# marja-w/gan-des-midi-music-gen

Measured on AMD Instinct MI355X. Metric: GAN training samples/sec (G+D step), higher is better.
Workload: dtype bf16; 1 GPU; SIMNN G/D iteration, synthetic 128x256 spectrogram windows; per_gpu_batch=256, global_batch=256, mode=faithful, parallelism=dp1

## Files before the change

### gan_des_midi_music_gen_amd/csrc/pointwise.hip

```cpp
#include "gdm_common.h"
#include "adam_pc.h"

namespace {

__global__ __launch_bounds__(1024) void bce_kernel(const float* __restrict__ x, float target, int n, float gscale,
                                                   float* __restrict__ loss, float* __restrict__ dx, int fuse_sig,
                                                   int accumulate) {
  __shared__ float red[1024];
  const int t = threadIdx.x;
  float s = 0.f;
  for (int i = t; i < n; i += 1024) {
    const float v = x[i];
    s += fmaxf(v, 0.f) - v * target + log1pf(expf(-fabsf(v)));
    if (dx) {
      float g = (1.0f / (1.0f + expf(-v)) - target) * gscale / (float)n;
      if (fuse_sig) g *= v * (1.f - v);
      dx[i] = g;
    }
  }
  red[t] = s;
  __syncthreads();
  for (int o = 512; o > 0; o >>= 1) {
    if (t < o) red[t] += red[t + o];
    __syncthreads();
// ... 67 lines not shown
                   blockIdx.z);
}

template <bool VEC>
__global__ __launch_bounds__(256) void adam_dev_kernel(float* __restrict__ p, const float* __restrict__ g,
                                                       float* __restrict__ m, float* __restrict__ v, int64_t n,
                                                       const float* __restrict__ hyper) {
  const float w1 = 1.0f - hyper[2], beta2 = hyper[3], omb2 = 1.0f - hyper[3], eps = hyper[4], gscale = hyper[5];
  const float step_size = hyper[6], bc2_sqrt = hyper[7];
  const int64_t stride = (int64_t)gridDim.x * 256 * 4;
  for (int64_t i = ((int64_t)blockIdx.x * 256 + threadIdx.x) * 4; i < n; i += stride) {
    if (VEC && i + 3 < n) {
      f32x4 pp = *(const f32x4*)(p + i), gg = *(const f32x4*)(g + i), mm = *(const f32x4*)(m + i),
            vv = *(const f32x4*)(v + i);
#pragma unroll
      for (int j = 0; j < 4; ++j) {
        float pj = pp[j], mj = mm[j], vj = vv[j];
        adam_element(pj, mj, vj, gg[j], gscale, w1, beta2, omb2, eps, step_size, bc2_sqrt);
        pp[j] = pj; mm[j] = mj; vv[j] = vj;
      }
      *(f32x4*)(p + i) = pp;
      *(f32x4*)(m + i) = mm;
      *(f32x4*)(v + i) = vv;
    } else {
      for (int64_t k = i; k < n && k < i + 4; ++k) {
        adam_element(p[k], m[k], v[k], g[k], gscale, w1, beta2, omb2, eps, step_size, bc2_sqrt);
      }
    }
  }
}

struct Welford { float n, mean, m2; };
__device__ __forceinline__ void welford_merge(Welford& a, const Welford& b) {
  if (b.n == 0.f) return;
  const float n = a.n + b.n;
  const float d = b.mean - a.mean;
  a.mean += d * (b.n / n);
  a.m2 += b.m2 + d * d * (a.n * b.n / n);
  a.n = n;
}

__device__ __forceinline__ Welford welford_from_shifted(float n, float shift, float s, float ss) {
  Welford a{n, 0.f, 0.f};
  if (n > 0.f) {
    a.mean = shift + s / n;
    a.m2 = fmaxf(ss - s * (s / n), 0.f);
  }
  return a;
}

__global__ __launch_bounds__(256) void bn_partial_stats(const float* __restrict__ y, int rows, int C, int chunk_rows,
                                                        int CW, float* __restrict__ ws) {
  __shared__ Welford sh[4][64];
  const int lane = threadIdx.x & 63, wv = threadIdx.x >> 6;
  const int rpl = 64 / CW;
  const int c = blockIdx.x * 64 + (lane & (CW - 1)), sub = lane / CW;
  const int r0 = blockIdx.y * chunk_rows, r1 = min(rows, r0 + chunk_rows);
  const int step = 4 * rpl;
  float n = 0.f, shift = 0.f, s = 0.f, ss = 0.f;
  if (c < C) {
    int r = r0 + wv * rpl + sub;
    if (r < r1) shift = y[(int64_t)r * C + c];
    for (; r + 7 * step < r1; r += 8 * step) {
      float x[8];
#pragma unroll
      for (int q = 0; q < 8; ++q) x[q] = y[(int64_t)(r + q * step) * C + c];
#pragma unroll
      for (int q = 0; q < 8; ++q) { const float d = x[q] - shift; s += d; ss += d * d; }
      n += 8.f;
    }
    for (; r < r1; r += step) { const float d = y[(int64_t)r * C + c] - shift; s += d; ss += d * d; n += 1.f; }
  }
  sh[wv][lane] = welford_from_shifted(n, shift, s, ss);
  __syncthreads();
  if (wv == 0 && sub == 0 && c < C) {
    Welford t{0.f, 0.f, 0.f};
    for (int w = 0; w < 4; ++w)
      for (int q = 0; q < rpl; ++q) welford_merge(t, sh[w][q * CW + lane]);
    float* o = ws + ((int64_t)blockIdx.y * C + c) * 3;
    o[0] = t.n; o[1] = t.mean; o[2] = t.m2;
  }
}

__global__ __launch_bounds__(1024) void bn_finalize(const float* __restrict__ ws, int chunks, int rows, int C,
                                                    float momentum, float eps, float* __restrict__ running_mean,
                                                    float* __restrict__ running_var, int64_t* __restrict__ nbt,
                                                    float* __restrict__ save_mean, float* __restrict__ save_invstd) {
  __shared__ Welford part[16][64];
  const int lane = threadIdx.x & 63, wv = threadIdx.x >> 6;
  const int c = blockIdx.x * 64 + lane;
  if (blockIdx.x == 0 && threadIdx.x == 0 && nbt) nbt[0] += 1;
  Welford t{0.f, 0.f, 0.f};
  if (c < C)
    for (int k = wv; k < chunks; k += 16 * 8) {
      Welford b[8];
#pragma unroll
      for (int q = 0; q < 8; ++q) {
        const int kk = k + 16 * q;
        const float* o = ws + ((int64_t)min(kk, chunks - 1) * C + c) * 3;
        b[q] = Welford{kk < chunks ? o[0] : 0.f, o[1], o[2]};
      }
#pragma unroll
      for (int q = 0; q < 8; ++q) welford_merge(t, b[q]);
    }
  part[wv][lane] = t;
  __syncthreads();
  if (wv != 0 || c >= C) return;
  t = part[0][lane];
#pragma unroll
  for (int w = 1; w < 16; ++w) welford_merge(t, part[w][lane]);
  const float var_b = t.m2 / (float)rows;
  save_mean[c] = t.mean;
  save_invstd[c] = 1.0f / sqrtf(var_b + eps);
  if (running_mean) {
    const float var_u = t.m2 / (float)max(rows - 1, 1);
    running_mean[c] = (1.f - momentum) * running_mean[c] + momentum * t.mean;
    running_var[c] = (1.f - momentum) * running_var[c] + momentum * var_u;
  }
}

__global__ __launch_bounds__(256) void bn_eval_stats(const float* __restrict__ running_mean,
                                                     const float* __restrict__ running_var, int C, float eps,
                                                     float* __restrict__ save_mean, float* __restrict__ save_invstd) {
  const int c = blockIdx.x * 256 + threadIdx.x;
  if (c >= C) return;
  save_mean[c] = running_mean[c];
  save_invstd[c] = 1.0f / sqrtf(running_var[c] + eps);
}

template <typename IT>
__global__ __launch_bounds__(256) void bn_apply(const float* __restrict__ y, int64_t total64, int C,
                                                const float* __restrict__ gamma, const float* __restrict__ beta,
                                                const float* __restrict__ mean, const float* __restrict__ invstd,
                                                int act, void* __restrict__ out, int out_dtype) {
  const IT total = (IT)total64, stride = (IT)gridDim.x * 256;
  for (IT i = (IT)blockIdx.x * 256 + threadIdx.x; i < total; i += stride) {
    const int c = (int)(i % C);
    const float alpha = invstd[c] * gamma[c];
    const float v = (y[i] - mean[c]) * alpha + beta[c];
    store_from_f32(out, out_dtype, i, apply_act(v, act, 0.f));
  }
}

__global__ __launch_bounds__(256) void bn_bwd_partial(const void* __restrict__ dout, const void* __restrict__ out,
                                                      int dtype, const float* __restrict__ y, int rows, int C,
                                                      int chunk_rows, const float* __restrict__ mean,
                                                      const float* __restrict__ invstd, int act,
                                                      float* __restrict__ ws) {
  __shared__ float sh1[4][64], sh2[4][64];
  const int lane = threadIdx.x & 63, wv = threadIdx.x >> 6;
  const int c = blockIdx.x * 64 + lane;
  const int r0 = blockIdx.y * chunk_rows, r1 = min(rows, r0 + chunk_rows);
  float s1 = 0.f, s2 = 0.f;
  if (c < C) {
    const float mu = mean[c], is = invstd[c];
    for (int r = r0 + wv; r < r1; r += 4) {
      const int64_t i = (int64_t)r * C + c;
      const float g = load_as_f32(dout, dtype, i) * act_grad_from_out(load_as_f32(out, dtype, i), act, 0.f);
      s1 += g;
      s2 += g * ((y[i] - mu) * is);
    }
  }
  sh1[wv][lane] = s1; sh2[wv][lane] = s2;
  __syncthreads();
  if (wv == 0 && c < C) {
    float* o = ws + ((int64_t)blockIdx.y * C + c) * 2;
    o[0] = ((sh1[0][lane] + sh1[1][lane]) + sh1[2][lane]) + sh1[3][lane];
    o[1] = ((sh2[0][lane] + sh2[1][lane]) + sh2[2][lane]) + sh2[3][lane];
  }
}

__global__ __launch_bounds__(256) void bn_bwd_finalize(const float* __restrict__ ws, int chunks, int C,
                                                       float* __restrict__ dgamma, float* __restrict__ dbeta) {
  const int c = blockIdx.x * 256 + threadIdx.x;
  if (c >= C) return;
  float s1 = 0.f, s2 = 0.f;
  for (int k = 0; k < chunks; ++k) {
    s1 += ws[((int64_t)k * C + c) * 2];
    s2 += ws[((int64_t)k * C + c) * 2 + 1];
  }
  dbeta[c] = s1;
  dgamma[c] = s2;
}

__global__ __launch_bounds__(256) void bn_bwd_apply(const void* __restrict__ dout, const void* __restrict__ out,
                                                    int dtype, const float* __restrict__ y, int64_t total, int rows,
                                                    int C, const float* __restrict__ gamma,
                                                    const float* __restrict__ mean, const float* __restrict__ invstd,
                                                    const float* __restrict__ dgamma, const float* __restrict__ dbeta,
                                                    int act, float* __restrict__ dy) {
  const int64_t stride = (int64_t)gridDim.x * 256;
  const float inv_r = 1.0f / (float)rows;
  for (int64_t i = (int64_t)blockIdx.x * 256 + threadIdx.x; i < total; i += stride) {
    const int c = (int)(i % C);
    const float g = load_as_f32(dout, dtype, i) * act_grad_from_out(load_as_f32(out, dtype, i), act, 0.f);
    const float xhat = (y[i] - mean[c]) * invstd[c];
    dy[i] = gamma[c] * invstd[c] * (g - dbeta[c] * inv_r - xhat * dgamma[c] * inv_r);
  }
}

__global__ __launch_bounds__(256) void bias_act_kernel(const float* __restrict__ x, const float* __restrict__ bias,
// ... 86 lines not shown
  GDM_LAUNCH_OK("gdm_criterion_loss");
  return GDM_OK;
}

extern "C" int gdm_adam_step(float* p, const float* g, float* m, float* v, int64_t n, int step, float lr, float beta1,
                             float beta2, float eps, float grad_scale, void* stream) {
  GDM_REQUIRE(p && g && m && v, "gdm_adam_step: null pointer");
  GDM_REQUIRE(n > 0 && step >= 1, "gdm_adam_step: bad n=%lld or step=%d", (long long)n, step);
  const bool aligned = (((uintptr_t)p | (uintptr_t)g | (uintptr_t)m | (uintptr_t)v) & 15) == 0;
  const double bc1 = 1.0 - pow((double)beta1, (double)step);
  const double bc2 = 1.0 - pow((double)beta2, (double)step);
  const float step_size = (float)((double)lr / bc1);
  const float bc2_sqrt = (float)sqrt(bc2);
  int64_t blocks = (n / 4 + 255) / 256;
  if (blocks < 1) blocks = 1;
  if (blocks > 8192) blocks = 8192;
  if (aligned)
    hipLaunchKernelGGL(adam_kernel<true>, dim3((unsigned)blocks), dim3(256), 0, (hipStream_t)stream, p, g, m, v, n,
                       1.0f - beta1, beta2, 1.0f - beta2, step_size, bc2_sqrt, eps, grad_scale);
  else
    hipLaunchKernelGGL(adam_kernel<false>, dim3((unsigned)blocks), dim3(256), 0, (hipStream_t)stream, p, g, m, v, n,
                       1.0f - beta1, beta2, 1.0f - beta2, step_size, bc2_sqrt, eps, grad_scale);
  GDM_LAUNCH_OK("gdm_adam_step");
  return GDM_OK;
}

extern "C" int gdm_adam_step_dev_pc(float* p, const float* g_pc, float* m, float* v, int N, int C, int P,
                                    void* shadow_pc, int shadow_dtype, float* hyper, int advance_step, void* stream) {
  GDM_REQUIRE(p && g_pc && m && v && shadow_pc && hyper, "gdm_adam_step_dev_pc: null pointer");
  GDM_REQUIRE(N > 0 && C > 0 && P > 0 && N <= 65535 && (C + 31) / 32 <= 65535 && gdm_dtype_ok(shadow_dtype),
              "gdm_adam_step_dev_pc: bad arguments");
  hipStream_t s = (hipStream_t)stream;
  if (advance_step) hipLaunchKernelGGL(adam_prep_kernel, dim3(1), dim3(1), 0, s, hyper);
  const dim3 grid((P + 127) / 128, (C + 31) / 32, N);
  const int vec_ok = (P % 4 == 0) && ((((uintptr_t)p | (uintptr_t)m | (uintptr_t)v) & 15) == 0);
  if (shadow_dtype == GDM_BF16)
    hipLaunchKernelGGL(adam_dev_pc_kernel<__bf16>, grid, dim3(256), 0, s, p, g_pc, m, v, C, P, (__bf16*)shadow_pc, hyper,
                       vec_ok);
  else
    hipLaunchKernelGGL(adam_dev_pc_kernel<float>, grid, dim3(256), 0, s, p, g_pc, m, v, C, P, (float*)shadow_pc, hyper,
                       vec_ok);
  GDM_LAUNCH_OK("gdm_adam_step_dev_pc");
  return GDM_OK;
}

extern "C" int gdm_adam_step_dev(float* p, const float* g, float* m, float* v, int64_t n, float* hyper, void* stream) {
  GDM_REQUIRE(p && g && m && v && hyper && n > 0, "gdm_adam_step_dev: bad arguments");
  const bool aligned = (((uintptr_t)p | (uintptr_t)g | (uintptr_t)m | (uintptr_t)v) & 15) == 0;
  int64_t blocks = (n / 4 + 255) / 256;
  if (blocks < 1) blocks = 1;
  if (blocks > 8192) blocks = 8192;
  hipStream_t s = (hipStream_t)stream;
  hipLaunchKernelGGL(adam_prep_kernel, dim3(1), dim3(1), 0, s, hyper);
  if (aligned) hipLaunchKernelGGL(adam_dev_kernel<true>, dim3((unsigned)blocks), dim3(256), 0, s, p, g, m, v, n, hyper);
  else hipLaunchKernelGGL(adam_dev_kernel<false>, dim3((unsigned)blocks), dim3(256), 0, s, p, g, m, v, n, hyper);
  GDM_LAUNCH_OK("gdm_adam_step_dev");
  return GDM_OK;
}

extern "C" size_t gdm_bn_workspace_bytes(int rows, int channels) {
  return (size_t)row_chunks(rows) * (size_t)channels * 3 * sizeof(float);
}

extern "C" int gdm_bn_act_fwd(const float* y, int rows, int channels, const float* gamma, const float* beta,
                              float* running_mean, float* running_var, int64_t* num_batches_tracked, float momentum,
                              float eps, int act, void* out, int out_dtype, float* save_mean, float* save_invstd,
                              int training, void* workspace, size_t workspace_bytes, void* stream) {
  GDM_REQUIRE(y && gamma && beta && out && save_mean && save_invstd, "gdm_bn_act_fwd: null pointer");
  GDM_REQUIRE(rows > 0 && channels > 0 && gdm_dtype_ok(out_dtype), "gdm_bn_act_fwd: bad arguments");
  hipStream_t s = (hipStream_t)stream;
  const int C = channels;
  if (training) {
    GDM_REQUIRE(rows > 1, "gdm_bn_act_fwd: training-mode batch norm needs more than 1 value per channel");
    const int chunks = row_chunks(rows);
    if (!workspace || workspace_bytes < gdm_bn_workspace_bytes(rows, C)) {
      gdm_set_error("gdm_bn_act_fwd: workspace too small");
      return GDM_EWORKSPACE;
    }
    const int chunk_rows = (rows + chunks - 1) / chunks;
    int cw = 64;
    while (cw / 2 >= C && cw > 1) cw /= 2;
    hipLaunchKernelGGL(bn_partial_stats, dim3((C + 63) / 64, chunks), dim3(256), 0, s, y, rows, C, chunk_rows, cw,
                       (float*)workspace);
    hipLaunchKernelGGL(bn_finalize, dim3((C + 63) / 64), dim3(1024), 0, s, (const float*)workspace, chunks, rows, C,
                       momentum, eps, running_mean, running_var, num_batches_tracked, save_mean, save_invstd);
  } else {
    GDM_REQUIRE(running_mean && running_var, "gdm_bn_act_fwd: eval mode needs running statistics");
    hipLaunchKernelGGL(bn_eval_stats, dim3((C + 255) / 256), dim3(256), 0, s, running_mean, running_var, C, eps,
                       save_mean, save_invstd);
  }
  const int64_t total = (int64_t)rows * C;
  if (total < ((int64_t)1 << 31))
    hipLaunchKernelGGL(bn_apply<int>, dim3(grid_for(total)), dim3(256), 0, s, y, total, C, gamma, beta, save_mean,
                       save_invstd, act, out, out_dtype);
  else
    hipLaunchKernelGGL(bn_apply<int64_t>, dim3(grid_for(total)), dim3(256), 0, s, y, total, C, gamma, beta, save_mean,
                       save_invstd, act, out, out_dtype);
  GDM_LAUNCH_OK("gdm_bn_act_fwd");
  return GDM_OK;
}

extern "C" int gdm_bn_partial_chunks(int rows) { return row_chunks(rows); }

extern "C" int gdm_bn_partials(const float* y, int rows, int channels, float* partials, void* stream) {
  GDM_REQUIRE(y && partials && rows > 0 && channels > 0, "gdm_bn_partials: bad arguments");
  const int C = channels, chunks = row_chunks(rows), chunk_rows = (rows + chunks - 1) / chunks;
  int cw = 64;
  while (cw / 2 >= C && cw > 1) cw /= 2;
  hipLaunchKernelGGL(bn_partial_stats, dim3((C + 63) / 64, chunks), dim3(256), 0, (hipStream_t)stream, y, rows, C,
                     chunk_rows, cw, partials);
  GDM_LAUNCH_OK("gdm_bn_partials");
  return GDM_OK;
}

extern "C" int gdm_bn_apply(const float* y, int rows, int channels, const float* gamma, const float* beta,
                            const float* mean, const float* invstd, int act, void* out, int out_dtype, void* stream) {
  GDM_REQUIRE(y && gamma && beta && mean && invstd && out && rows > 0 && channels > 0 && gdm_dtype_ok(out_dtype),
              "gdm_bn_apply: bad arguments");
  const int64_t total = (int64_t)rows * channels;
  hipStream_t s = (hipStream_t)stream;
  if (total < ((int64_t)1 << 31))
    hipLaunchKernelGGL(bn_apply<int>, dim3(grid_for(total)), dim3(256), 0, s, y, total, channels, gamma, beta, mean, invstd,
                       act, out, out_dtype);
  else
    hipLaunchKernelGGL(bn_apply<int64_t>, dim3(grid_for(total)), dim3(256), 0, s, y, total, channels, gamma, beta, mean,
                       invstd, act, out, out_dtype);
  GDM_LAUNCH_OK("gdm_bn_apply");
  return GDM_OK;
}

extern "C" int gdm_bn_finalize(const float* ws, int chunks, int rows, int channels, float momentum, float eps,
                               float* running_mean, float* running_var, int64_t* num_batches_tracked, float* save_mean,
                               float* save_invstd, void* stream) {
  GDM_REQUIRE(ws && save_mean && save_invstd && chunks > 0 && rows > 1 && channels > 0, "gdm_bn_finalize: bad arguments");
  hipLaunchKernelGGL(bn_finalize, dim3((channels + 63) / 64), dim3(1024), 0, (hipStream_t)stream, ws, chunks, rows,
                     channels, momentum, eps, running_mean, running_var, num_batches_tracked, save_mean, save_invstd);
  GDM_LAUNCH_OK("gdm_bn_finalize");
  return GDM_OK;
}

extern "C" int gdm_bn_stats(const float* y, int rows, int channels, float* running_mean, float* running_var,
                            int64_t* num_batches_tracked, float momentum, float eps, float* save_mean,
                            float* save_invstd, void* workspace, size_t workspace_bytes, void* stream) {
  GDM_REQUIRE(y && save_mean && save_invstd && rows > 1 && channels > 0, "gdm_bn_stats: bad arguments");
  if (!workspace || workspace_bytes < gdm_bn_workspace_bytes(rows, channels)) {
    gdm_set_error("gdm_bn_stats: workspace too small");
    return GDM_EWORKSPACE;
  }
  hipStream_t s = (hipStream_t)stream;
  const int C = channels, chunks = row_chunks(rows), chunk_rows = (rows + chunks - 1) / chunks;
  int cw = 64;
  while (cw / 2 >= C && cw > 1) cw /= 2;
  hipLaunchKernelGGL(bn_partial_stats, dim3((C + 63) / 64, chunks), dim3(256), 0, s, y, rows, C, chunk_rows, cw,
                     (float*)workspace);
  hipLaunchKernelGGL(bn_finalize, dim3((C + 63) / 64), dim3(1024), 0, s, (const float*)workspace, chunks, rows, C,
                     momentum, eps, running_mean, running_var, num_batches_tracked, save_mean, save_invstd);
  GDM_LAUNCH_OK("gdm_bn_stats");
  return GDM_OK;
}

extern "C" int gdm_bn_act_bwd(const void* dout, const void* out, int out_dtype, const float* y, int rows, int channels,
                              const float* gamma, const float* save_mean, const float* save_invstd, int act,
                              float* dy, float* dgamma, float* dbeta, void* workspace, size_t workspace_bytes,
                              void* stream) {
  GDM_REQUIRE(dout && out && y && gamma && save_mean && save_invstd && dy && dgamma && dbeta,
              "gdm_bn_act_bwd: null pointer");
  GDM_REQUIRE(rows > 0 && channels > 0 && gdm_dtype_ok(out_dtype), "gdm_bn_act_bwd: bad arguments");
  const int C = channels, chunks = row_chunks(rows);
  if (!workspace || workspace_bytes < gdm_bn_workspace_bytes(rows, C)) {
    gdm_set_error("gdm_bn_act_bwd: workspace too small");
    return GDM_EWORKSPACE;
  }
  hipStream_t s = (hipStream_t)stream;
  const int chunk_rows = (rows + chunks - 1) / chunks;
  hipLaunchKernelGGL(bn_bwd_partial, dim3((C + 63) / 64, chunks), dim3(256), 0, s, dout, out, out_dtype, y, rows, C,
                     chunk_rows, save_mean, save_invstd, act, (float*)workspace);
  hipLaunchKernelGGL(bn_bwd_finalize, dim3((C + 255) / 256), dim3(256), 0, s, (const float*)workspace, chunks, C,
                     dgamma, dbeta);
  const int64_t total = (int64_t)rows * C;
  hipLaunchKernelGGL(bn_bwd_apply, dim3(grid_for(total)), dim3(256), 0, s, dout, out, out_dtype, y, total, rows, C,
                     gamma, save_mean, save_invstd, dgamma, dbeta, act, dy);
  GDM_LAUNCH_OK("gdm_bn_act_bwd");
  return GDM_OK;
}

extern "C" int gdm_bias_act_fwd(const float* x, const float* bias, int rows, int cols, int act, float slope, void* out,
                                int out_dtype, void* stream) {
  GDM_REQUIRE(x && out && rows > 0 && cols > 0 && gdm_dtype_ok(out_dtype), "gdm_bias_act_fwd: bad arguments");
  const int64_t total = (int64_t)rows * cols;
  hipLaunchKernelGGL(bias_act_kernel, dim3(grid_for(total)), dim3(256), 0, (hipStream_t)stream, x, bias, total, cols,
                     act, slope, out, out_dtype);
  GDM_LAUNCH_OK("gdm_bias_act_fwd");
  return GDM_OK;
}

extern "C" int gdm_act_bwd(const void* dout, const void* out, int dtype, int64_t n, int act, float slope, void* dx,
                           void* stream) {
  GDM_REQUIRE(dout && out && dx && n > 0 && gdm_dtype_ok(dtype), "gdm_act_bwd: bad arguments");
  hipLaunchKernelGGL(act_bwd_kernel, dim3(grid_for(n)), dim3(256), 0, (hipStream_t)stream, dout, out, dtype, n, act,
                     slope, dx);
  GDM_LAUNCH_OK("gdm_act_bwd");
  return GDM_OK;
}

extern "C" int gdm_colsum(const void* x, int dtype, int rows, int cols, float* out, void* workspace,
                          size_t workspace_bytes, void* stream) {
  GDM_REQUIRE(x && out && rows > 0 && cols > 0 && gdm_dtype_ok(dtype), "gdm_colsum: bad arguments");
  const int chunks = row_chunks(rows);
  if (!workspace || workspace_bytes < (size_t)chunks * cols * sizeof(float)) {
    gdm_set_error("gdm_colsum: workspace too small (need %zu)", (size_t)chunks * cols * sizeof(float));
    return GDM_EWORKSPACE;
  }
  hipStream_t s = (hipStream_t)stream;
  const int chunk_rows = (rows + chunks - 1) / chunks;
  hipLaunchKernelGGL(colsum_partial, dim3((cols + 63) / 64, chunks), dim3(256), 0, s, x, dtype, rows, cols, chunk_rows,
                     (float*)workspace);
  hipLaunchKernelGGL(colsum_final, dim3((cols + 255) / 256), dim3(256), 0, s, (const float*)workspace, chunks, cols,
                     out);
  GDM_LAUNCH_OK("gdm_colsum");
  return GDM_OK;
}

extern "C" int gdm_cast(const void* src, int src_dtype, void* dst, int dst_dtype, int64_t n, void* stream) {
  GDM_REQUIRE(src && dst && n > 0 && gdm_dtype_ok(src_dtype) && gdm_dtype_ok(dst_dtype), "gdm_cast: bad arguments");
  hipLaunchKernelGGL(cast_kernel, dim3(grid_for(n)), dim3(256), 0, (hipStream_t)stream, src, src_dtype, dst,
                     dst_dtype, n);
  GDM_LAUNCH_OK("gdm_cast");
  return GDM_OK;
}

namespace {
constexpr int HEAD_ROWS = 8;
__global__ __launch_bounds__(256) void simnn_head_kernel(const float* __restrict__ h1, const float* __restrict__ w2,
                                                         const float* __restrict__ b2, int n, int n0, float y0,
                                                         float y1, float* __restrict__ prob, void* __restrict__ dh1,
                                                         int dh1_bf16, float* __restrict__ partials) {
  __shared__ float dz_s[HEAD_ROWS], lt_s[HEAD_ROWS], part[2][256];
  const int t = threadIdx.x, lane = t & 63, wv = t >> 6;
  const int r0 = blockIdx.x * HEAD_ROWS, r1 = min(n, r0 + HEAD_ROWS);
// ... 171 lines not shown
```

### gan_des_midi_music_gen_amd/csrc/simnn_gen.hip

```cpp
#include "buffer_ops.h"

namespace {

template <int CIN, int COUT>
__device__ __forceinline__ void pack_one(const float* __restrict__ w, __bf16* __restrict__ dst, int i) {
  constexpr int K = 4 * CIN;
  const int k = i % K, co = (i / K) % COUT, cl = i / (K * COUT);
  const int ci = k % CIN, t = k / CIN, a = t >> 1, b = t & 1, qy = cl >> 1, qx = cl & 1;
  const int kh = 1 - qy + 2 * a, kw = 1 - qx + 2 * b;
  dst[i] = (__bf16)w[((ci * COUT + co) * 4 + kh) * 4 + kw];
}
constexpr int GP_W2 = 4 * 64 * 4 * 128, GP_W3 = 4 * 32 * 4 * 64;
constexpr int L1_K = 128, GP_W1 = 16 * 128 * L1_K;
__global__ __launch_bounds__(256) void gen_pack_kernel(const float* __restrict__ w1, int noise_dim,
                                                       const float* __restrict__ w2, const float* __restrict__ w3,
                                                       __bf16* __restrict__ pack) {
  const int i = blockIdx.x * 256 + threadIdx.x;
  if (i < GP_W2) pack_one<128, 64>(w2, pack, i);
  else if (i < GP_W2 + GP_W3) pack_one<64, 32>(w3, pack + GP_W2, i - GP_W2);
  else if (i < GP_W2 + GP_W3 + GP_W1) {
    const int j = i - GP_W2 - GP_W3, k = j % L1_K, n = j / L1_K, co = n % 128, pos = n / 128;
    pack[i] = (__bf16)(k < noise_dim ? w1[((size_t)k * 128 + co) * 16 + pos] : 0.f);
  }
}

constexpr int L1_CH = 4;
__global__ __launch_bounds__(256) void gen_l1_kernel(const float* __restrict__ noise, int B, int noise_dim,
                                                     const __bf16* __restrict__ w1p, float* __restrict__ y1,
                                                     float momentum, float eps, float* __restrict__ running_mean,
                                                     float* __restrict__ running_var, int64_t* __restrict__ nbt,
                                                     float* __restrict__ save_mean, float* __restrict__ save_invstd) {
  constexpr int SK = L1_K + 8;
  extern __shared__ __attribute__((aligned(16))) unsigned char dyn_smem[];
  __bf16* x_s = (__bf16*)dyn_smem;
  __bf16* w_s = x_s + 256 * SK;
  __shared__ float red[4][L1_CH], cmean[L1_CH];
  const int t = threadIdx.x, l = t & 63, wv = t >> 6, lr = l & 15, lg = l >> 4;
  const int c0 = blockIdx.x * L1_CH;
  {
    f32x4 wr[4];
#pragma unroll
    for (int k = 0; k < 4; ++k) {
      const int i = t + 256 * k, row = i / (L1_K / 8), c8 = i % (L1_K / 8), pos = row >> 2, co = row & 3;
      wr[k] = *(const f32x4*)&w1p[((size_t)(pos * 128 + c0 + co)) * L1_K + 8 * c8];
    }
    const bool vec = (noise_dim % 4 == 0) && (((uintptr_t)noise & 15) == 0);
#pragma unroll
    for (int half = 0; half < 2; ++half) {
      f32x4 xr[16];
#pragma unroll
      for (int k = 0; k < 16; ++k) {
        const int i = t + 256 * (k + 16 * half), b = i / (L1_K / 4), k4 = 4 * (i % (L1_K / 4));
        xr[k] = (f32x4){0.f, 0.f, 0.f, 0.f};
        if (b < B && k4 < noise_dim) {
          const float* src = noise + (size_t)b * noise_dim + k4;
          if (vec) xr[k] = *(const f32x4*)src;
          else
#pragma unroll
            for (int e = 0; e < 4; ++e) xr[k][e] = (k4 + e < noise_dim) ? src[e] : 0.f;
        }
      }
      if (half == 0) {
#pragma unroll
        for (int k = 0; k < 4; ++k) {
          const int i = t + 256 * k, row = i / (L1_K / 8), c8 = i % (L1_K / 8);
          *(f32x4*)&w_s[row * SK + 8 * c8] = wr[k];
        }
      }
#pragma unroll
      for (int k = 0; k < 16; ++k) {
        const int i = t + 256 * (k + 16 * half), b = i / (L1_K / 4), k4 = 4 * (i % (L1_K / 4));
        bf16x4 h;
#pragma unroll
        for (int e = 0; e < 4; ++e) h[e] = (__bf16)xr[k][e];
        *(bf16x4*)&x_s[b * SK + k4] = h;
      }
    }
  }
  __syncthreads();
  f32x4 acc[16];
#pragma unroll
  for (int bt = 0; bt < 16; ++bt) acc[bt] = (f32x4){0.f, 0.f, 0.f, 0.f};
#pragma unroll
  for (int ks = 0; ks < L1_K / 32; ++ks) {
    const bf16x8 af = *(const bf16x8*)&w_s[(16 * wv + lr) * SK + ks * 32 + 8 * lg];
#pragma unroll
    for (int bt = 0; bt < 16; ++bt) {
      const bf16x8 bf = *(const bf16x8*)&x_s[(bt * 16 + lr) * SK + ks * 32 + 8 * lg];
      acc[bt] = mfma16(af, bf, acc[bt]);
    }
  }
#pragma unroll
  for (int bt = 0; bt < 16; ++bt) {
    const int b = bt * 16 + lr;
    if (b < B) *(f32x4*)&y1[((size_t)b * 16 + 4 * wv + lg) * 128 + c0] = acc[bt];
  }
  auto reduce = [&](auto value) {
#pragma unroll
    for (int r = 0; r < L1_CH; ++r) {
      float sum = 0.f;
#pragma unroll
      for (int bt = 0; bt < 16; ++bt) sum += (bt * 16 + lr < B) ? value(acc[bt][r], r) : 0.f;
      sum += __shfl_xor(sum, 1, 64); sum += __shfl_xor(sum, 2, 64); sum += __shfl_xor(sum, 4, 64);
      sum += __shfl_xor(sum, 8, 64); sum += __shfl_xor(sum, 16, 64); sum += __shfl_xor(sum, 32, 64);
      if (l == 0) red[wv][r] = sum;
    }
  };
  const float n = (float)B * 16.f;
  reduce([&](float v, int) { return v; });
  __syncthreads();
  if (t < L1_CH) cmean[t] = (((red[0][t] + red[1][t]) + red[2][t]) + red[3][t]) / n;
  __syncthreads();
  reduce([&](float v, int c) { const float d = v - cmean[c]; return d * d; });
  __syncthreads();
  if (t < L1_CH) {
    const float m2 = ((red[0][t] + red[1][t]) + red[2][t]) + red[3][t];
    const int c = c0 + t;
    save_mean[c] = cmean[t];
    save_invstd[c] = 1.0f / sqrtf(m2 / n + eps);
    if (running_mean) {
      running_mean[c] = (1.f - momentum) * running_mean[c] + momentum * cmean[t];
      running_var[c] = (1.f - momentum) * running_var[c] + momentum * (m2 / fmaxf(n - 1.f, 1.f));
    }
  }
  if (blockIdx.x == 0 && t == 0 && nbt) nbt[0] += 1;
}

template <int CIN, int COUT, int IH, int S>
__global__ __launch_bounds__(256) void convt_s2_bn_kernel(const float* __restrict__ yin, const float* __restrict__ mean,
                                                          const float* __restrict__ invstd,
                                                          const float* __restrict__ gamma,
                                                          const float* __restrict__ beta, int B,
                                                          const __bf16* __restrict__ wp, float* __restrict__ yout,
                                                          float* __restrict__ ws) {
  constexpr int K = 4 * CIN, HP = IH + 2, NPX = S * IH * IH, PT = NPX / 16, CT = COUT / 16, OH = 2 * IH;
  constexpr int TILES = PT * CT, TPW = TILES / 4;
  constexpr int SIN = CIN + 8, SW = K + 8;
  static_assert(NPX % 16 == 0 && TILES % 4 == 0 && CIN % 32 == 0, "tile shapes");
  extern __shared__ __attribute__((aligned(16))) unsigned char dyn_smem[];
  __bf16* in_s = (__bf16*)dyn_smem;
  __bf16* w_s = in_s + S * HP * HP * SIN;
  float* red = (float*)(w_s + COUT * SW);
  __shared__ float sm[CIN], sc[CIN], sh[CIN], cmean[COUT];
  const int t = threadIdx.x, l = t & 63, wv = t >> 6, lr = l & 15, lg = l >> 4;
  const int cl = blockIdx.x & 3, grp = blockIdx.x >> 2, qy = cl >> 1, qx = cl & 1;
  const int s0 = grp * S;
  for (int c = t; c < CIN; c += 256) {
    sm[c] = mean[c];
    sc[c] = invstd[c] * gamma[c];
    sh[c] = beta[c];
  }
  constexpr int WV = COUT * K / 8 / 256, XV = S * IH * IH * (CIN / 4) / 256;
  static_assert((COUT * K / 8) % 256 == 0 && (S * IH * IH * (CIN / 4)) % 256 == 0, "staging loops are exact");
  f32x4 wr[WV], xr[XV];
#pragma unroll
  for (int k = 0; k < WV; ++k) wr[k] = ((const f32x4*)(wp + (size_t)cl * COUT * K))[t + 256 * k];
#pragma unroll
  for (int k = 0; k < XV; ++k) {
    const int i = t + 256 * k, c4 = i % (CIN / 4), px = i / (CIN / 4), s = px / (IH * IH);
    xr[k] = (f32x4){0.f, 0.f, 0.f, 0.f};
    if (s0 + s < B) xr[k] = *(const f32x4*)(yin + ((size_t)s0 * IH * IH + px) * CIN + 4 * c4);
  }
  for (int i = t; i < S * HP * HP * SIN / 8; i += 256) ((f32x4*)in_s)[i] = (f32x4){0.f, 0.f, 0.f, 0.f};
#pragma unroll
  for (int k = 0; k < WV; ++k) {
    const int i = t + 256 * k, row = i / (K / 8), c8 = i % (K / 8);
    *(f32x4*)&w_s[row * SW + 8 * c8] = wr[k];
  }
  __syncthreads();
#pragma unroll
  for (int k = 0; k < XV; ++k) {
    const int i = t + 256 * k, c4 = i % (CIN / 4), px = i / (CIN / 4), s = px / (IH * IH), iy = (px / IH) % IH, ix = px % IH;
    bf16x4 h;
#pragma unroll
    for (int e = 0; e < 4; ++e)
      h[e] = (__bf16)fmaxf((xr[k][e] - sm[4 * c4 + e]) * sc[4 * c4 + e] + sh[4 * c4 + e], 0.f);
    if (s0 + s < B) *(bf16x4*)&in_s[((s * HP + iy + 1) * HP + ix + 1) * SIN + 4 * c4] = h;
  }
  __syncthreads();
  f32x4 acc[TPW];
#pragma unroll
  for (int q = 0; q < TPW; ++q) acc[q] = (f32x4){0.f, 0.f, 0.f, 0.f};
  constexpr int PTW = TPW / CT;
  int boff[PTW];
#pragma unroll
  for (int p = 0; p < PTW; ++p) {
    const int px = (wv * PTW + p) * 16 + lr, s = px / (IH * IH), i = (px / IH) % IH, j = px % IH;
    boff[p] = ((s * HP + i + qy + 1) * HP + j + qx + 1) * SIN;
  }
#pragma unroll 2
  for (int ks = 0; ks < K / 32; ++ks) {
    const int tap = (ks * 32) / CIN, ci0 = (ks * 32) % CIN, a = tap >> 1, b = tap & 1;
    bf16x8 af[CT], bf[PTW];
#pragma unroll
    for (int c = 0; c < CT; ++c) af[c] = *(const bf16x8*)&w_s[(c * 16 + lr) * SW + ks * 32 + 8 * lg];
#pragma unroll
    for (int p = 0; p < PTW; ++p) bf[p] = *(const bf16x8*)&in_s[boff[p] - (a * HP + b) * SIN + ci0 + 8 * lg];
#pragma unroll
    for (int p = 0; p < PTW; ++p)
#pragma unroll
      for (int c = 0; c < CT; ++c) acc[p * CT + c] = mfma16(af[c], bf[p], acc[p * CT + c]);
  }
#pragma unroll
  for (int p = 0; p < PTW; ++p) {
    const int px = (wv * PTW + p) * 16 + lr, s = px / (IH * IH), i = (px / IH) % IH, j = px % IH;
    if (s0 + s < B) {
      float* dst = yout + ((size_t)(s0 + s) * OH * OH + (2 * i + qy) * OH + 2 * j + qx) * COUT + 4 * lg;
#pragma unroll
      for (int c = 0; c < CT; ++c) *(f32x4*)(dst + 16 * c) = acc[p * CT + c];
    }
  }
  const int n_valid = min(S, max(0, B - s0)) * IH * IH;
  auto reduce = [&](auto value) {
#pragma unroll
    for (int c = 0; c < CT; ++c)
#pragma unroll
      for (int r = 0; r < 4; ++r) {
        float sum = 0.f;
#pragma unroll
        for (int p = 0; p < PTW; ++p) {
          const int px = (wv * PTW + p) * 16 + lr;
          sum += (s0 + px / (IH * IH) < B) ? value(acc[p * CT + c][r], 16 * c + 4 * lg + r) : 0.f;
        }
        sum += __shfl_xor(sum, 1, 64); sum += __shfl_xor(sum, 2, 64);
        sum += __shfl_xor(sum, 4, 64); sum += __shfl_xor(sum, 8, 64);
        if (lr == 0) red[wv * COUT + 16 * c + 4 * lg + r] = sum;
      }
  };
  reduce([&](float v, int) { return v; });
  __syncthreads();
  if (t < COUT) cmean[t] = (((red[t] + red[COUT + t]) + red[2 * COUT + t]) + red[3 * COUT + t]) / (float)max(n_valid, 1);
  __syncthreads();
  reduce([&](float v, int co) { const float d = v - cmean[co]; return d * d; });
  __syncthreads();
  if (t < COUT) {
    const float m2 = ((red[t] + red[COUT + t]) + red[2 * COUT + t]) + red[3 * COUT + t];
    float* o = ws + ((size_t)blockIdx.x * COUT + t) * 3;
    o[0] = (float)n_valid; o[1] = cmean[t]; o[2] = m2;
  }
}

__global__ __launch_bounds__(512) void convt_k5_bn_sigmoid_kernel(const float* __restrict__ yin,
                                                                  const float* __restrict__ mean,
                                                                  const float* __restrict__ invstd,
                                                                  const float* __restrict__ gamma,
                                                                  const float* __restrict__ beta,
                                                                  const float* __restrict__ w4, float* __restrict__ out) {
  constexpr int C = 32, IH = 16, OH = 20, SP = C + 4;
  __shared__ __attribute__((aligned(16))) float in_s[IH * IH * SP];
  __shared__ __attribute__((aligned(16))) float w_s[25 * C];
  __shared__ float sm[C], sc[C], sh[C];
  const int t = threadIdx.x, b = blockIdx.x;
  if (t < C) {
    sm[t] = mean[t];
    sc[t] = invstd[t] * gamma[t];
    sh[t] = beta[t];
  }
  for (int i = t; i < 25 * C; i += 512) w_s[i] = w4[(i % C) * 25 + i / C];
  __syncthreads();
  const f32x4* src = (const f32x4*)(yin + (size_t)b * IH * IH * C);
  for (int i = t; i < IH * IH * C / 4; i += 512) {
    f32x4 v = src[i];
    const int c4 = (i % (C / 4)) * 4;
#pragma unroll
    for (int e = 0; e < 4; ++e) v[e] = fmaxf((v[e] - sm[c4 + e]) * sc[c4 + e] + sh[c4 + e], 0.f);
    *(f32x4*)&in_s[(i / (C / 4)) * SP + c4] = v;
  }
  __syncthreads();
  const int o = t;
  if (o < OH * OH) {
    const int oy = o / OH, ox = o % OH;
    float a0 = 0.f, a1 = 0.f, a2 = 0.f, a3 = 0.f;
#pragma unroll 1
    for (int kh = 0; kh < 5; ++kh) {
      const int iy = oy - kh;
      if ((unsigned)iy >= (unsigned)IH) continue;
#pragma unroll 1
      for (int kw = 0; kw < 5; ++kw) {
        const int ix = ox - kw;
        if ((unsigned)ix >= (unsigned)IH) continue;
        const f32x4* xp = (const f32x4*)&in_s[(iy * IH + ix) * SP];
        const f32x4* wq = (const f32x4*)&w_s[(kh * 5 + kw) * C];
#pragma unroll
        for (int q = 0; q < C / 4; ++q) {
          const f32x4 xv = xp[q], wv = wq[q];
          a0 = fmaf(xv[0], wv[0], a0); a1 = fmaf(xv[1], wv[1], a1);
          a2 = fmaf(xv[2], wv[2], a2); a3 = fmaf(xv[3], wv[3], a3);
        }
      }
    }
    out[(size_t)b * OH * OH + o] = sigmoid_f((a0 + a1) + (a2 + a3));
  }
}

struct gen_eval_params {
  const float* noise;
  int B, noise_dim;
  const __bf16* pack;
  const float* w4;
  const float *gamma1, *beta1, *rmean1, *rvar1, *gamma2, *beta2, *rmean2, *rvar2, *gamma3, *beta3, *rmean3, *rvar3;
  float eps;
  float* out;
  float *tap_y1, *tap_y2, *tap_y3, *tap_invstd;
};

template <bool TAPS>
__global__ __launch_bounds__(512) void gen_eval_kernel(const gen_eval_params p) {
  constexpr int S1 = 128 + 8, S2 = 64 + 8, S3 = 32 + 4, NC = 128 + 64 + 32;
  __shared__ __attribute__((aligned(16))) unsigned char r0[256 * S3 * 4];
  __shared__ __attribute__((aligned(16))) __bf16 a2[10 * 10 * S2];
  __shared__ __attribute__((aligned(16))) float w_s[25 * 32];
  __shared__ float sm[NC], sc[NC], sh[NC];
  static_assert(6 * 6 * S1 * 2 <= (int)sizeof(r0) && (6 * 6 * S1 * 2) % 16 == 0 && (10 * 10 * S2 * 2) % 16 == 0, "LDS images");
  __bf16* a1 = (__bf16*)r0;
  float* a3 = (float*)r0;
  const int t = threadIdx.x, l = t & 63, wv = t >> 6, lr = l & 15, lg = l >> 4;
  const int b = blockIdx.x;
  if (t < NC) {
    const int c = t < 128 ? t : (t < 192 ? t - 128 : t - 192);
    const float* gamma = t < 128 ? p.gamma1 : (t < 192 ? p.gamma2 : p.gamma3);
    const float* beta = t < 128 ? p.beta1 : (t < 192 ? p.beta2 : p.beta3);
    const float* rmean = t < 128 ? p.rmean1 : (t < 192 ? p.rmean2 : p.rmean3);
    const float* rvar = t < 128 ? p.rvar1 : (t < 192 ? p.rvar2 : p.rvar3);
    const float invstd = 1.0f / sqrtf(rvar[c] + p.eps);
    sm[t] = rmean[c];
    sc[t] = invstd * gamma[c];
    sh[t] = beta[c];
    if (TAPS && b == 0 && p.tap_invstd) p.tap_invstd[t] = invstd;
  }
  for (int i = t; i < 25 * 32; i += 512) w_s[i] = p.w4[(i % 32) * 25 + i / 32];
  for (int i = t; i < 6 * 6 * S1 / 8; i += 512) ((f32x4*)a1)[i] = (f32x4){0.f, 0.f, 0.f, 0.f};
  for (int i = t; i < 10 * 10 * S2 / 8; i += 512) ((f32x4*)a2)[i] = (f32x4){0.f, 0.f, 0.f, 0.f};
  bf16x8 nf[L1_K / 32];
#pragma unroll
  for (int ks = 0; ks < L1_K / 32; ++ks)
#pragma unroll
    for (int j = 0; j < 8; ++j) {
      const int k = ks * 32 + 8 * lg + j;
      nf[ks][j] = (__bf16)((lr == 0 && k < p.noise_dim) ? p.noise[(size_t)b * p.noise_dim + k] : 0.f);
    }
  __syncthreads();
  auto stage4 = [&](const f32x4& v, int ch) {
    f32x4 r;
#pragma unroll
    for (int e = 0; e < 4; ++e) r[e] = fmaxf(__builtin_fmaf(v[e] - sm[ch + e], sc[ch + e], sh[ch + e]), 0.f);
    return r;
  };
  auto to_bf16x4 = [](const f32x4& v) {
    bf16x4 h;
#pragma unroll
    for (int e = 0; e < 4; ++e) h[e] = (__bf16)v[e];
    return h;
  };
  {
    const __bf16* w1p = p.pack + GP_W2 + GP_W3;
#pragma unroll 8
    for (int q = 0; q < 16; ++q) {
      const int tile = wv * 16 + q;
      const __bf16* row = w1p + (size_t)(tile * 16 + lr) * L1_K + 8 * lg;
      bf16x8 af[L1_K / 32];
#pragma unroll
      for (int ks = 0; ks < L1_K / 32; ++ks) af[ks] = *(const bf16x8*)(row + ks * 32);
      f32x4 acc = (f32x4){0.f, 0.f, 0.f, 0.f};
#pragma unroll
      for (int ks = 0; ks < L1_K / 32; ++ks) acc = mfma16(af[ks], nf[ks], acc);
      if (lr == 0) {
        const int pos = tile >> 3, co = (tile & 7) * 16 + 4 * lg;
        if (TAPS && p.tap_y1) *(f32x4*)&p.tap_y1[((size_t)b * 16 + pos) * 128 + co] = acc;
        *(bf16x4*)&a1[(((pos >> 2) + 1) * 6 + (pos & 3) + 1) * S1 + co] = to_bf16x4(stage4(acc, co));
      }
    }
  }
  __syncthreads();
  const int cl = wv & 3, mh = wv >> 2, qy = cl >> 1, qx = cl & 1;
// ... 39 lines not shown
    }
    const int co = mh * 16 + 4 * lg;
#pragma unroll
    for (int pt = 0; pt < 4; ++pt) {
      const int px = pt * 16 + lr, oy = 2 * (px >> 3) + qy, ox = 2 * (px & 7) + qx;
      if (TAPS && p.tap_y3) *(f32x4*)&p.tap_y3[((size_t)b * 256 + oy * 16 + ox) * 32 + co] = acc[pt];
      *(f32x4*)&a3[(oy * 16 + ox) * S3 + co] = stage4(acc[pt], 192 + co);
    }
  }
  __syncthreads();
  if (t < 400) {
    const int oy = t / 20, ox = t % 20;
    float s0 = 0.f, s1 = 0.f, s2 = 0.f, s3 = 0.f;
#pragma unroll 1
    for (int kh = 0; kh < 5; ++kh) {
      const int iy = oy - kh;
      if ((unsigned)iy >= 16u) continue;
#pragma unroll 1
      for (int kw = 0; kw < 5; ++kw) {
        const int ix = ox - kw;
        if ((unsigned)ix >= 16u) continue;
        const f32x4* xp = (const f32x4*)&a3[(iy * 16 + ix) * S3];
        const f32x4* wq = (const f32x4*)&w_s[(kh * 5 + kw) * 32];
#pragma unroll
        for (int q = 0; q < 8; ++q) {
          const f32x4 xv = xp[q], wq4 = wq[q];
          s0 = fmaf(xv[0], wq4[0], s0); s1 = fmaf(xv[1], wq4[1], s1);
          s2 = fmaf(xv[2], wq4[2], s2); s3 = fmaf(xv[3], wq4[3], s3);
        }
      }
    }
    p.out[(size_t)b * 400 + t] = sigmoid_f((s0 + s1) + (s2 + s3));
  }
}

template <int CIN, int COUT, int IH, int S>
int launch_convt_s2(const float* yin, const float* mean, const float* invstd, const float* gamma, const float* beta,
                    int B, const __bf16* wp, float* yout, float* ws, hipStream_t s) {
  const size_t sm = ((size_t)S * (IH + 2) * (IH + 2) * (CIN + 8) + (size_t)COUT * (4 * CIN + 8)) * 2 + (size_t)4 * COUT * 4;
  allow_lds(convt_s2_bn_kernel<CIN, COUT, IH, S>, sm);
  const int groups = (B + S - 1) / S;
  hipLaunchKernelGGL((convt_s2_bn_kernel<CIN, COUT, IH, S>), dim3(4 * groups), dim3(256), sm, s, yin, mean, invstd, gamma,
                     beta, B, wp, yout, ws);
  return 4 * groups;
}

}

extern "C" size_t gdm_simnn_gen_pack_bytes(void) { return (size_t)(GP_W2 + GP_W3 + GP_W1) * 2; }

extern "C" int gdm_simnn_gen_pack(const float* w1, int noise_dim, const float* w2, const float* w3, void* pack,
                                  void* stream) {
  GDM_REQUIRE(w1 && w2 && w3 && pack && ((uintptr_t)pack & 15) == 0 && noise_dim >= 1 && noise_dim <= L1_K,
              "gdm_simnn_gen_pack: bad arguments (noise_dim <= %d)", L1_K);
  hipLaunchKernelGGL(gen_pack_kernel, dim3((GP_W2 + GP_W3 + GP_W1 + 255) / 256), dim3(256), 0, (hipStream_t)stream, w1,
                     noise_dim, w2, w3, (__bf16*)pack);
  GDM_LAUNCH_OK("gdm_simnn_gen_pack");
  return GDM_OK;
}

extern "C" int gdm_simnn_gen_first(const float* noise, int B, int noise_dim, const void* pack, float* y1, float momentum,
                                   float eps, float* running_mean, float* running_var, int64_t* num_batches_tracked,
                                   float* save_mean, float* save_invstd, void* stream) {
  GDM_REQUIRE(noise && pack && y1 && save_mean && save_invstd, "gdm_simnn_gen_first: null pointer");
  GDM_REQUIRE(B > 1 && B <= 256 && noise_dim >= 1 && noise_dim <= L1_K && ((uintptr_t)y1 & 15) == 0,
              "gdm_simnn_gen_first: batch %d outside 2..256 (the workgroup owns the whole batch) or noise_dim > %d", B, L1_K);
  const size_t sm = (size_t)(256 + 16 * L1_CH) * (L1_K + 8) * 2;
  allow_lds(gen_l1_kernel, sm);
  hipLaunchKernelGGL(gen_l1_kernel, dim3(128 / L1_CH), dim3(256), sm, (hipStream_t)stream, noise, B, noise_dim,
                     (const __bf16*)pack + GP_W2 + GP_W3, y1, momentum, eps, running_mean, running_var,
                     num_batches_tracked, save_mean, save_invstd);
  GDM_LAUNCH_OK("gdm_simnn_gen_first");
  return GDM_OK;
}

extern "C" int gdm_simnn_gen_convt_chunks(int layer, int B) { return layer == 2 ? 4 * ((B + 7) / 8) : 4 * ((B + 3) / 4); }

extern "C" int gdm_simnn_gen_convt_bn(int layer, const float* yin, const float* mean, const float* invstd,
                                      const float* gamma, const float* beta, int B, const void* pack, float* yout,
                                      float* ws_partials, void* stream) {
  GDM_REQUIRE(yin && mean && invstd && gamma && beta && pack && yout && ws_partials && B > 0 && (layer == 2 || layer == 3),
              "gdm_simnn_gen_convt_bn: bad arguments");
  GDM_REQUIRE((((uintptr_t)yin | (uintptr_t)yout | (uintptr_t)pack) & 15) == 0, "gdm_simnn_gen_convt_bn: 16-byte alignment");
  hipStream_t s = (hipStream_t)stream;
  if (layer == 2) launch_convt_s2<128, 64, 4, 8>(yin, mean, invstd, gamma, beta, B, (const __bf16*)pack, yout, ws_partials, s);
  else launch_convt_s2<64, 32, 8, 4>(yin, mean, invstd, gamma, beta, B, (const __bf16*)pack + GP_W2, yout, ws_partials, s);
  GDM_LAUNCH_OK("gdm_simnn_gen_convt_bn");
  return GDM_OK;
}

extern "C" int gdm_simnn_gen_last(const float* yin, const float* mean, const float* invstd, const float* gamma,
                                  const float* beta, const float* w4, int B, float* out, void* stream) {
  GDM_REQUIRE(yin && mean && invstd && gamma && beta && w4 && out && B > 0 && ((uintptr_t)yin & 15) == 0,
              "gdm_simnn_gen_last: bad arguments");
  hipLaunchKernelGGL(convt_k5_bn_sigmoid_kernel, dim3(B), dim3(512), 0, (hipStream_t)stream, yin, mean, invstd, gamma,
                     beta, w4, out);
  GDM_LAUNCH_OK("gdm_simnn_gen_last");
  return GDM_OK;
}

extern "C" int gdm_simnn_gen_eval(const float* noise, int B, int noise_dim, const void* pack, const float* w4,
                                  const float* gamma1, const float* beta1, const float* rmean1, const float* rvar1,
                                  const float* gamma2, const float* beta2, const float* rmean2, const float* rvar2,
                                  const float* gamma3, const float* beta3, const float* rmean3, const float* rvar3,
                                  float eps, float* out, float* tap_y1, float* tap_y2, float* tap_y3, float* tap_invstd,
                                  void* stream) {
  GDM_REQUIRE(noise && pack && w4 && out, "gdm_simnn_gen_eval: null pointer");
  GDM_REQUIRE(gamma1 && beta1 && rmean1 && rvar1 && gamma2 && beta2 && rmean2 && rvar2 && gamma3 && beta3 && rmean3 && rvar3,
              "gdm_simnn_gen_eval: null BatchNorm vector");
  GDM_REQUIRE(B >= 1 && noise_dim >= 1 && noise_dim <= L1_K, "gdm_simnn_gen_eval: batch %d < 1 or noise_dim %d outside 1..%d",
              B, noise_dim, L1_K);
  GDM_REQUIRE(eps >= 0.f, "gdm_simnn_gen_eval: eps < 0");
  GDM_REQUIRE(((uintptr_t)pack & 15) == 0 && ((uintptr_t)out & 15) == 0 && ((uintptr_t)noise & 3) == 0 &&
                  (((uintptr_t)tap_y1 | (uintptr_t)tap_y2 | (uintptr_t)tap_y3) & 15) == 0 && ((uintptr_t)tap_invstd & 3) == 0,
              "gdm_simnn_gen_eval: alignment (pack, out and the taps 16 bytes, noise 4)");
  gen_eval_params p;
  p.noise = noise; p.B = B; p.noise_dim = noise_dim; p.pack = (const __bf16*)pack; p.w4 = w4;
  p.gamma1 = gamma1; p.beta1 = beta1; p.rmean1 = rmean1; p.rvar1 = rvar1;
  p.gamma2 = gamma2; p.beta2 = beta2; p.rmean2 = rmean2; p.rvar2 = rvar2;
  p.gamma3 = gamma3; p.beta3 = beta3; p.rmean3 = rmean3; p.rvar3 = rvar3;
  p.eps = eps; p.out = out;
  p.tap_y1 = tap_y1; p.tap_y2 = tap_y2; p.tap_y3 = tap_y3; p.tap_invstd = tap_invstd;
  if (tap_y1 || tap_y2 || tap_y3 || tap_invstd)
    hipLaunchKernelGGL(gen_eval_kernel<true>, dim3(B), dim3(512), 0, (hipStream_t)stream, p);
  else
    hipLaunchKernelGGL(gen_eval_kernel<false>, dim3(B), dim3(512), 0, (hipStream_t)stream, p);
  GDM_LAUNCH_OK("gdm_simnn_gen_eval");
  return GDM_OK;
}
```

Before: 428,900 samples/s.

## Shrink BN finalize blocks, buffer-load staging, and hoist loads in generator kernels

Templates bn_finalize on channel width and launches it with 16-channel blocks (256 threads) instead of 64-channel 1024-thread blocks, which spreads small-C finalization over more workgroups. The generator layer-1 and strided convT kernels now use buffer loads with out-of-bounds masking and issue all global loads before LDS stores. The k5 sigmoid kernel hoists its input loads ahead of the weight staging and uses packed 2-wide FMAs. The aim is to hide global-load latency and cut per-kernel overhead, at the cost of extra register pressure and a new batch-size limit for buffer addressing.

```diff
diff --git a/gan_des_midi_music_gen_amd/csrc/pointwise.hip b/gan_des_midi_music_gen_amd/csrc/pointwise.hip
--- a/gan_des_midi_music_gen_amd/csrc/pointwise.hip
+++ b/gan_des_midi_music_gen_amd/csrc/pointwise.hip
@@ -173,13 +173,14 @@
   }
 }
 
-__global__ __launch_bounds__(1024) void bn_finalize(const float* __restrict__ ws, int chunks, int rows, int C,
-                                                    float momentum, float eps, float* __restrict__ running_mean,
-                                                    float* __restrict__ running_var, int64_t* __restrict__ nbt,
-                                                    float* __restrict__ save_mean, float* __restrict__ save_invstd) {
-  __shared__ Welford part[16][64];
-  const int lane = threadIdx.x & 63, wv = threadIdx.x >> 6;
-  const int c = blockIdx.x * 64 + lane;
+template <int CW>
+__global__ __launch_bounds__(16 * CW) void bn_finalize(const float* __restrict__ ws, int chunks, int rows, int C,
+                                                       float momentum, float eps, float* __restrict__ running_mean,
+                                                       float* __restrict__ running_var, int64_t* __restrict__ nbt,
+                                                       float* __restrict__ save_mean, float* __restrict__ save_invstd) {
+  __shared__ Welford part[16][CW];
+  const int lane = threadIdx.x % CW, wv = threadIdx.x / CW;
+  const int c = blockIdx.x * CW + lane;
   if (blockIdx.x == 0 && threadIdx.x == 0 && nbt) nbt[0] += 1;
   Welford t{0.f, 0.f, 0.f};
   if (c < C)
@@ -208,6 +209,14 @@
     running_mean[c] = (1.f - momentum) * running_mean[c] + momentum * t.mean;
     running_var[c] = (1.f - momentum) * running_var[c] + momentum * var_u;
   }
+}
+
+constexpr int BNF_CW = 16;
+inline void launch_bn_finalize(hipStream_t s, const float* ws, int chunks, int rows, int C, float momentum, float eps,
+                               float* running_mean, float* running_var, int64_t* nbt, float* save_mean,
+                               float* save_invstd) {
+  hipLaunchKernelGGL(bn_finalize<BNF_CW>, dim3((C + BNF_CW - 1) / BNF_CW), dim3(16 * BNF_CW), 0, s, ws, chunks, rows, C,
+                     momentum, eps, running_mean, running_var, nbt, save_mean, save_invstd);
 }
 
 __global__ __launch_bounds__(256) void bn_eval_stats(const float* __restrict__ running_mean,
@@ -460,8 +469,8 @@
     while (cw / 2 >= C && cw > 1) cw /= 2;
     hipLaunchKernelGGL(bn_partial_stats, dim3((C + 63) / 64, chunks), dim3(256), 0, s, y, rows, C, chunk_rows, cw,
                        (float*)workspace);
-    hipLaunchKernelGGL(bn_finalize, dim3((C + 63) / 64), dim3(1024), 0, s, (const float*)workspace, chunks, rows, C,
-                       momentum, eps, running_mean, running_var, num_batches_tracked, save_mean, save_invstd);
+    launch_bn_finalize(s, (const float*)workspace, chunks, rows, C, momentum, eps, running_mean, running_var,
+                       num_batches_tracked, save_mean, save_invstd);
   } else {
     GDM_REQUIRE(running_mean && running_var, "gdm_bn_act_fwd: eval mode needs running statistics");
     hipLaunchKernelGGL(bn_eval_stats, dim3((C + 255) / 256), dim3(256), 0, s, running_mean, running_var, C, eps,
@@ -511,8 +520,8 @@
                                float* running_mean, float* running_var, int64_t* num_batches_tracked, float* save_mean,
                                float* save_invstd, void* stream) {
   GDM_REQUIRE(ws && save_mean && save_invstd && chunks > 0 && rows > 1 && channels > 0, "gdm_bn_finalize: bad arguments");
-  hipLaunchKernelGGL(bn_finalize, dim3((channels + 63) / 64), dim3(1024), 0, (hipStream_t)stream, ws, chunks, rows,
-                     channels, momentum, eps, running_mean, running_var, num_batches_tracked, save_mean, save_invstd);
+  launch_bn_finalize((hipStream_t)stream, ws, chunks, rows, channels, momentum, eps, running_mean, running_var,
+                     num_batches_tracked, save_mean, save_invstd);
   GDM_LAUNCH_OK("gdm_bn_finalize");
   return GDM_OK;
 }
@@ -531,8 +540,8 @@
   while (cw / 2 >= C && cw > 1) cw /= 2;
   hipLaunchKernelGGL(bn_partial_stats, dim3((C + 63) / 64, chunks), dim3(256), 0, s, y, rows, C, chunk_rows, cw,
                      (float*)workspace);
-  hipLaunchKernelGGL(bn_finalize, dim3((C + 63) / 64), dim3(1024), 0, s, (const float*)workspace, chunks, rows, C,
-                     momentum, eps, running_mean, running_var, num_batches_tracked, save_mean, save_invstd);
+  launch_bn_finalize(s, (const float*)workspace, chunks, rows, C, momentum, eps, running_mean, running_var,
+                     num_batches_tracked, save_mean, save_invstd);
   GDM_LAUNCH_OK("gdm_bn_stats");
   return GDM_OK;
 }
diff --git a/gan_des_midi_music_gen_amd/csrc/simnn_gen.hip b/gan_des_midi_music_gen_amd/csrc/simnn_gen.hip
--- a/gan_des_midi_music_gen_amd/csrc/simnn_gen.hip
+++ b/gan_des_midi_music_gen_amd/csrc/simnn_gen.hip
@@ -45,35 +45,49 @@
       wr[k] = *(const f32x4*)&w1p[((size_t)(pos * 128 + c0 + co)) * L1_K + 8 * c8];
     }
     const bool vec = (noise_dim % 4 == 0) && (((uintptr_t)noise & 15) == 0);
-#pragma unroll
-    for (int half = 0; half < 2; ++half) {
-      f32x4 xr[16];
-#pragma unroll
-      for (int k = 0; k < 16; ++k) {
-        const int i = t + 256 * (k + 16 * half), b = i / (L1_K / 4), k4 = 4 * (i % (L1_K / 4));
-        xr[k] = (f32x4){0.f, 0.f, 0.f, 0.f};
-        if (b < B && k4 < noise_dim) {
-          const float* src = noise + (size_t)b * noise_dim + k4;
-          if (vec) xr[k] = *(const f32x4*)src;
-          else
+    auto stage_w = [&]() {
+#pragma unroll
+      for (int k = 0; k < 4; ++k) {
+        const int i = t + 256 * k, row = i / (L1_K / 8), c8 = i % (L1_K / 8);
+        *(f32x4*)&w_s[row * SK + 8 * c8] = wr[k];
+      }
+    };
+    auto stage_x = [&](int k, const f32x4& x) {
+      const int i = t + 256 * k, b = i / (L1_K / 4), k4 = 4 * (i % (L1_K / 4));
+      bf16x4 h;
+#pragma unroll
+      for (int e = 0; e < 4; ++e) h[e] = (__bf16)x[e];
+      *(bf16x4*)&x_s[b * SK + k4] = h;
+    };
+    if (vec) {
+      const rsrc_t nr = make_rsrc(noise, (uint32_t)B * (uint32_t)noise_dim * 4u);
+      f32x4 xr[32];
+#pragma unroll
+      for (int k = 0; k < 32; ++k) {
+        const int i = t + 256 * k, b = i / (L1_K / 4), k4 = 4 * (i % (L1_K / 4));
+        xr[k] = buf_load16(nr, b < B && k4 < noise_dim ? (uint32_t)((b * noise_dim + k4) * 4) : BUF_OOB);
+      }
+      __builtin_amdgcn_sched_barrier(0);
+      stage_w();
+#pragma unroll
+      for (int k = 0; k < 32; ++k) stage_x(k, xr[k]);
+    } else {
+#pragma unroll
+      for (int half = 0; half < 2; ++half) {
+        f32x4 xr[16];
+#pragma unroll
+        for (int k = 0; k < 16; ++k) {
+          const int i = t + 256 * (k + 16 * half), b = i / (L1_K / 4), k4 = 4 * (i % (L1_K / 4));
+          xr[k] = (f32x4){0.f, 0.f, 0.f, 0.f};
+          if (b < B && k4 < noise_dim) {
+            const float* src = noise + (size_t)b * noise_dim + k4;
 #pragma unroll
             for (int e = 0; e < 4; ++e) xr[k][e] = (k4 + e < noise_dim) ? src[e] : 0.f;
+          }
         }
-      }
-      if (half == 0) {
-#pragma unroll
-        for (int k = 0; k < 4; ++k) {
-          const int i = t + 256 * k, row = i / (L1_K / 8), c8 = i % (L1_K / 8);
-          *(f32x4*)&w_s[row * SK + 8 * c8] = wr[k];
-        }
-      }
-#pragma unroll
-      for (int k = 0; k < 16; ++k) {
-        const int i = t + 256 * (k + 16 * half), b = i / (L1_K / 4), k4 = 4 * (i % (L1_K / 4));
-        bf16x4 h;
-#pragma unroll
-        for (int e = 0; e < 4; ++e) h[e] = (__bf16)xr[k][e];
-        *(bf16x4*)&x_s[b * SK + k4] = h;
+        if (half == 0) stage_w();
+#pragma unroll
+        for (int k = 0; k < 16; ++k) stage_x(k + 16 * half, xr[k]);
       }
     }
   }
@@ -145,27 +159,30 @@
   const int t = threadIdx.x, l = t & 63, wv = t >> 6, lr = l & 15, lg = l >> 4;
   const int cl = blockIdx.x & 3, grp = blockIdx.x >> 2, qy = cl >> 1, qx = cl & 1;
   const int s0 = grp * S;
-  for (int c = t; c < CIN; c += 256) {
-    sm[c] = mean[c];
-    sc[c] = invstd[c] * gamma[c];
-    sh[c] = beta[c];
-  }
+  static_assert(CIN <= 256, "one BatchNorm channel per thread");
+  const int cb = min(t, CIN - 1);
+  const float bn_mean = mean[cb], bn_invstd = invstd[cb], bn_gamma = gamma[cb], bn_beta = beta[cb];
   constexpr int WV = COUT * K / 8 / 256, XV = S * IH * IH * (CIN / 4) / 256;
   static_assert((COUT * K / 8) % 256 == 0 && (S * IH * IH * (CIN / 4)) % 256 == 0, "staging loops are exact");
   f32x4 wr[WV], xr[XV];
 #pragma unroll
   for (int k = 0; k < WV; ++k) wr[k] = ((const f32x4*)(wp + (size_t)cl * COUT * K))[t + 256 * k];
+  const rsrc_t yr = make_rsrc(yin, (uint32_t)B * (IH * IH * CIN * 4));
 #pragma unroll
   for (int k = 0; k < XV; ++k) {
     const int i = t + 256 * k, c4 = i % (CIN / 4), px = i / (CIN / 4), s = px / (IH * IH);
-    xr[k] = (f32x4){0.f, 0.f, 0.f, 0.f};
-    if (s0 + s < B) xr[k] = *(const f32x4*)(yin + ((size_t)s0 * IH * IH + px) * CIN + 4 * c4);
+    xr[k] = buf_load16(yr, s0 + s < B ? (uint32_t)(((s0 * IH * IH + px) * CIN + 4 * c4) * 4) : BUF_OOB);
   }
   for (int i = t; i < S * HP * HP * SIN / 8; i += 256) ((f32x4*)in_s)[i] = (f32x4){0.f, 0.f, 0.f, 0.f};
 #pragma unroll
   for (int k = 0; k < WV; ++k) {
     const int i = t + 256 * k, row = i / (K / 8), c8 = i % (K / 8);
     *(f32x4*)&w_s[row * SW + 8 * c8] = wr[k];
+  }
+  if (t < CIN) {
+    sm[t] = bn_mean;
+    sc[t] = bn_invstd * bn_gamma;
+    sh[t] = bn_beta;
   }
   __syncthreads();
 #pragma unroll
@@ -250,7 +267,13 @@
   __shared__ __attribute__((aligned(16))) float in_s[IH * IH * SP];
   __shared__ __attribute__((aligned(16))) float w_s[25 * C];
   __shared__ float sm[C], sc[C], sh[C];
+  typedef float f32x2 __attribute__((ext_vector_type(2)));
   const int t = threadIdx.x, b = blockIdx.x;
+  constexpr int XV = IH * IH * C / 4 / 512;
+  const f32x4* src = (const f32x4*)(yin + (size_t)b * IH * IH * C);
+  f32x4 xr[XV];
+#pragma unroll
+  for (int k = 0; k < XV; ++k) xr[k] = src[t + 512 * k];
   if (t < C) {
     sm[t] = mean[t];
     sc[t] = invstd[t] * gamma[t];
@@ -258,10 +281,10 @@
   }
   for (int i = t; i < 25 * C; i += 512) w_s[i] = w4[(i % C) * 25 + i / C];
   __syncthreads();
-  const f32x4* src = (const f32x4*)(yin + (size_t)b * IH * IH * C);
-  for (int i = t; i < IH * IH * C / 4; i += 512) {
-    f32x4 v = src[i];
-    const int c4 = (i % (C / 4)) * 4;
+#pragma unroll
+  for (int k = 0; k < XV; ++k) {
+    const int i = t + 512 * k, c4 = (i % (C / 4)) * 4;
+    f32x4 v = xr[k];
 #pragma unroll
     for (int e = 0; e < 4; ++e) v[e] = fmaxf((v[e] - sm[c4 + e]) * sc[c4 + e] + sh[c4 + e], 0.f);
     *(f32x4*)&in_s[(i / (C / 4)) * SP + c4] = v;
@@ -270,7 +293,7 @@
   const int o = t;
   if (o < OH * OH) {
     const int oy = o / OH, ox = o % OH;
-    float a0 = 0.f, a1 = 0.f, a2 = 0.f, a3 = 0.f;
+    f32x2 a01 = {0.f, 0.f}, a23 = {0.f, 0.f};
 #pragma unroll 1
     for (int kh = 0; kh < 5; ++kh) {
       const int iy = oy - kh;
@@ -284,12 +307,12 @@
 #pragma unroll
         for (int q = 0; q < C / 4; ++q) {
           const f32x4 xv = xp[q], wv = wq[q];
-          a0 = fmaf(xv[0], wv[0], a0); a1 = fmaf(xv[1], wv[1], a1);
-          a2 = fmaf(xv[2], wv[2], a2); a3 = fmaf(xv[3], wv[3], a3);
+          a01 = __builtin_elementwise_fma((f32x2){xv[0], xv[1]}, (f32x2){wv[0], wv[1]}, a01);
+          a23 = __builtin_elementwise_fma((f32x2){xv[2], xv[3]}, (f32x2){wv[2], wv[3]}, a23);
         }
       }
     }
-    out[(size_t)b * OH * OH + o] = sigmoid_f((a0 + a1) + (a2 + a3));
+    out[(size_t)b * OH * OH + o] = sigmoid_f((a01[0] + a01[1]) + (a23[0] + a23[1]));
   }
 }
 
@@ -495,6 +518,7 @@
   GDM_REQUIRE(yin && mean && invstd && gamma && beta && pack && yout && ws_partials && B > 0 && (layer == 2 || layer == 3),
               "gdm_simnn_gen_convt_bn: bad arguments");
   GDM_REQUIRE((((uintptr_t)yin | (uintptr_t)yout | (uintptr_t)pack) & 15) == 0, "gdm_simnn_gen_convt_bn: 16-byte alignment");
+  GDM_REQUIRE(B <= (1 << 16), "gdm_simnn_gen_convt_bn: batch %d > 65536 (the input is addressed through a 2-GiB buffer)", B);
   hipStream_t s = (hipStream_t)stream;
   if (layer == 2) launch_convt_s2<128, 64, 4, 8>(yin, mean, invstd, gamma, beta, B, (const __bf16*)pack, yout, ws_partials, s);
   else launch_convt_s2<64, 32, 8, 4>(yin, mean, invstd, gamma, beta, B, (const __bf16*)pack + GP_W2, yout, ws_partials, s);
```

Measured after the change: 430,000 samples/s (median of 2 runs). Within noise of the previous version (+0.3%).
